# PKU-EPIC/GraspNeRF

Hardware: AMD Instinct MI355X
Metric: scenes/sec TSDF+render fwd, 6-view 40^3 grid (higher is better)
Workload: dtype f32

## Files before the change

graspnerf_amd/_lib.py:

```python
import ctypes as C
import os

_HERE = os.path.dirname(os.path.abspath(__file__))
LIB_PATH = os.path.join(_HERE, 'csrc', os.environ.get('GNR_LIB', 'libgnr.so'))

GNR_OK, GNR_ERR_ARG, GNR_ERR_SHAPE, GNR_ERR_HIP, GNR_ERR_WORKSPACE = 0, -1, -2, -3, -4
ERRORS = {-1: 'GNR_ERR_ARG', -2: 'GNR_ERR_SHAPE', -3: 'GNR_ERR_HIP', -4: 'GNR_ERR_WORKSPACE'}

c_float_p = C.POINTER(C.c_float)


class GnrScene(C.Structure):
    _fields_ = [('B', C.c_int), ('V', C.c_int), ('H', C.c_int), ('W', C.c_int), ('fh', C.c_int), ('fw', C.c_int),
                ('imgs', C.c_void_p), ('img_feats', C.c_void_p), ('ray_feats', C.c_void_p),
                ('poses', C.c_void_p), ('Ks', C.c_void_p), ('depth_range', C.c_void_p), ('use_vis', C.c_int), ('options', C.c_uint)]


OPTIONS = {'fp32_chain': 0x001, 'feature_grad_fixed': 0x002, 'view1_one_wavefront': 0x004, 'view2_one_wavefront': 0x008,
           'ray_order_morton': 0x010, 'poison_partials': 0x020, 'direct_scatter': 0x040, 'geo_dual_fp32': 0x080, 'test_lose_partner': 0x100, 'static_tiles': 0x200, 'split_launch': 0x400}
GNR_STATUS_LOST_PARTNER = 16


class GnrRays(C.Structure):
    _fields_ = [('rn', C.c_int), ('dn', C.c_int), ('fdn', C.c_int),
                ('ray_mask_view_num', C.c_int), ('ray_mask_point_num', C.c_int),
                ('coords', C.c_void_p), ('que_pose', C.c_void_p), ('que_K', C.c_void_p),
                ('que_depth_range', C.c_void_p), ('que_imgs', C.c_void_p), ('fine_u', C.c_void_p),
                ('ray_batch_num', C.c_int), ('fine_depth_use_all', C.c_int)]


RENDER_OUT_FIELDS = ['depth', 'sdf_values', 'alpha_values', 'colors_nr', 'hit_prob_nr', 'pixel_colors_nr',
                     'pixel_colors_gt', 'render_depth', 'ray_mask', 'sdf_gradient_error', 'sdf_gradient', 'view_mask']


# ... 51 lines not shown
    L.gnr_status_words_offset.restype = C.c_size_t
    L.gnr_sample_volume_fwd.argtypes = [C.POINTER(GnrScene), C.c_void_p, C.c_int, C.c_void_p, C.c_void_p,
                                        C.c_void_p, C.c_void_p, C.c_size_t, C.c_void_p]
    L.gnr_sample_volume_fwd.restype = C.c_int
    L.gnr_debug_volume_chain.argtypes = [C.POINTER(GnrScene), C.c_void_p, C.c_int, C.c_void_p, C.c_void_p,
                                         C.c_void_p, C.c_size_t, C.c_void_p]
    L.gnr_debug_volume_chain.restype = C.c_int
    L.gnr_depth_mean_fwd.argtypes = [C.POINTER(GnrScene), C.c_void_p, C.c_int, C.c_void_p, C.c_void_p,
                                     C.c_void_p, C.c_size_t, C.c_void_p]
    L.gnr_depth_mean_fwd.restype = C.c_int
    L.gnr_merge_depths.argtypes = [C.c_void_p, C.c_int, C.c_void_p, C.c_int, C.c_void_p, C.c_int, C.c_void_p]
    L.gnr_merge_depths.restype = C.c_int
    L.gnr_render_by_depth_fwd.argtypes = [C.POINTER(GnrScene), C.POINTER(GnrRays), C.c_void_p, C.c_int, C.c_void_p,
                                          C.POINTER(GnrRenderOut), C.c_void_p, C.c_size_t, C.c_void_p]
    L.gnr_render_by_depth_fwd.restype = C.c_int
    L.gnr_render_rays_fwd.argtypes = [C.POINTER(GnrScene), C.POINTER(GnrRays), C.c_void_p, C.c_void_p,
                                      C.POINTER(GnrRenderOut), C.POINTER(GnrRenderOut), C.c_void_p, C.c_void_p,
                                      C.c_void_p, C.c_size_t, C.c_void_p]
    L.gnr_render_rays_fwd.restype = C.c_int
    L.gnr_head_canonical_floats.restype = C.c_int
    L.gnr_head_packed_floats.restype = C.c_int
    L.gnr_pack_grasp_head.argtypes = [c_float_p, c_float_p]
    L.gnr_pack_grasp_head.restype = C.c_int
    L.gnr_grasp_head_workspace_bytes.argtypes = [C.c_int, C.c_int]
    L.gnr_grasp_head_workspace_bytes.restype = C.c_size_t
    L.gnr_grasp_head_fwd.argtypes = [C.c_int, C.c_int, C.c_void_p, C.c_void_p, C.c_void_p, C.c_void_p, C.c_void_p,
                                     C.c_void_p, C.c_size_t, C.c_void_p]
    L.gnr_grasp_head_fwd.restype = C.c_int
    L.gnr_head_last_error.restype = C.c_char_p
    L.gnr_conv3d_bwd_weight.argtypes = [C.c_void_p] * 3 + [C.c_int] * 7 + [C.c_void_p]
# ... 88 lines not shown
    for fn in (L.gnr_reflect_pad2d, L.gnr_reflect_pad2d_bwd):
        fn.argtypes = [C.c_void_p, C.c_void_p, C.c_longlong, C.c_int, C.c_int, C.c_int, C.c_void_p]
        fn.restype = C.c_int
    L.gnr_upsample2x_bilinear.argtypes = [C.c_void_p, C.c_void_p, C.c_longlong, C.c_int, C.c_int, C.c_void_p]
    L.gnr_upsample2x_bilinear.restype = C.c_int
    L.gnr_last_error.restype = C.c_char_p
    L.gnr_dominant_kernel_name.restype = C.c_char_p
    L.gnr_debug_fill_lds.argtypes = [C.c_uint, C.c_void_p]
    L.gnr_debug_fill_lds.restype = C.c_int
    _lib = L
    return L


EXPORTED = ['gnr_canonical_weights_floats', 'gnr_packed_weights_floats', 'gnr_pack_weights', 'gnr_pack_vis_decoder', 'gnr_pack_vis_decoder_bwd', 'gnr_canonical_vis_floats', 'gnr_pack_weights_device', 'gnr_pack_weights_bwd_device', 'gnr_pack_vis_decoder_device', 'gnr_pack_vis_decoder_bwd_device', 'gnr_layout_offset', 'gnr_workspace_bytes',
            'gnr_prepare', 'gnr_range_status', 'gnr_status_words_offset', 'gnr_sample_volume_fwd', 'gnr_debug_volume_chain', 'gnr_depth_mean_fwd', 'gnr_merge_depths', 'gnr_render_by_depth_fwd', 'gnr_render_rays_fwd',
            'gnr_dominant_kernel_name', 'gnr_last_error', 'gnr_time_chain_kernel', 'gnr_head_canonical_floats',
            'gnr_head_packed_floats', 'gnr_pack_grasp_head', 'gnr_grasp_head_workspace_bytes', 'gnr_grasp_head_fwd',
            'gnr_head_last_error', 'gnr_chain_timing_begin', 'gnr_chain_timing_end', 'gnr_timing_begin', 'gnr_timing_begin_only', 'gnr_timing_end', 'gnr_grasp_select_workspace_bytes',
            'gnr_grasp_select_fwd', 'gnr_post_last_error', 'gnr_packed_bwd_floats', 'gnr_pack_weights_bwd',
            'gnr_depth_mean_bwd_workspace_bytes', 'gnr_depth_mean_bwd', 'gnr_sample_volume_train_workspace_bytes',
            'gnr_train_workspace_layout', 'gnr_sample_volume_fwd_train', 'gnr_sample_volume_bwd',
            'gnr_render_chain_train_workspace_bytes', 'gnr_render_chain_fwd_train', 'gnr_render_chain_bwd', 'gnr_conv3d_bwd_weight', 'gnr_conv3d_same_workspace_bytes', 'gnr_conv3d_same', 'gnr_conv3d_tap_mask_words', 'gnr_conv3d_tap_mask', 'gnr_conv3d_same_masked', 'gnr_conv3d_same_bwd_weight_masked', 'gnr_conv3d_same_bwd_weight', 'gnr_conv3d_same_bwd_weight_workspace_bytes',
            'gnr_render_tail_fwd_train', 'gnr_ray_tail_grad_floats', 'gnr_ray_tail_dual_bwd', 'gnr_ray_tail_dual_bwd_workspace_bytes', 'gnr_composite_bwd', 'gnr_composite_bwd_workspace_bytes', 'gnr_geo_dual_fwd', 'gnr_geo_dual_fwd_workspace_bytes', 'gnr_geo_dual_bwd', 'gnr_geo_dual_bwd_workspace_bytes', 'gnr_host_randperm_prefix',
            'gnr_debug_fill_lds', 'gnr_img_last_error', 'gnr_instnorm_act', 'gnr_instnorm_act_bwd', 'gnr_reflect_pad2d', 'gnr_reflect_pad2d_bwd', 'gnr_upsample2x_bilinear']


def check(rc, what):
    if rc != GNR_OK:
        msg = lib().gnr_last_error().decode(errors='replace')
        raise GnrError(f'{what} failed: {ERRORS.get(rc, rc)} ({msg})')
# ... 17 lines not shown
```

graspnerf_amd/csrc/gnr_capi.inc:

```
#include <stdio.h>
#include <string.h>
#include <atomic>
#include <mutex>

#include "../../include/gnr.h"

namespace gnr {

static thread_local char g_err[512] = "";
static int fail(int code, const char* what, hipError_t e = hipSuccess) {
    snprintf(g_err, sizeof(g_err), "%s%s%s", what, e != hipSuccess ? ": " : "", e != hipSuccess ? hipGetErrorString(e) : "");
    return code;
}
#define GNR_HIP(call)                                                         \
    do {                                                                      \
        hipError_t e_ = (call);                                               \
        if (e_ != hipSuccess) return fail(GNR_ERR_HIP, #call, e_);            \
    } while (0)

static inline size_t al256(size_t x) { return (x + 255) & ~(size_t)255; }

static bool attr_needed(std::atomic<unsigned long long>& done) {
    int dev = 0;
    if (hipGetDevice(&dev) != hipSuccess) return true;
    const unsigned long long bit = 1ull << (dev & 63);
    if (done.load() & bit) return false;
    done.fetch_or(bit);
    return true;
}

struct Workspace {
    float* feat64; float* viewp; unsigned* range_flag;
    float* desc; float* rec; float* depth_c; float* depth_f; float* depth_m; float* gerr_part; unsigned char* vmask_pts;
    int* ray_perm;
    size_t total;
};

static Workspace carve(const GnrScene* s, size_t P, size_t rn, void* base) {
    Workspace w;
    char* p = (char*)base;
    size_t off = 0;
    const size_t BV = (size_t)s->B * s->V;
    auto take = [&](size_t bytes) { char* q = p ? p + off : nullptr; off += al256(bytes); return q; };
    w.feat64 = (float*)take(BV * s->fh * s->fw * 64 * sizeof(float));
    w.viewp = (float*)take(BV * VIEWP_FLOATS * sizeof(float));
    w.range_flag = (unsigned*)take(512);
    w.desc = (float*)take((size_t)s->B * P * DESC_FLOATS * sizeof(float));
    w.rec = (float*)take((size_t)s->B * P * REC_RAY * sizeof(float));
    w.depth_c = (float*)take((size_t)s->B * P * sizeof(float));
    w.depth_f = (float*)take((size_t)s->B * P * sizeof(float));
    w.depth_m = (float*)take((size_t)s->B * P * sizeof(float));
    w.gerr_part = (float*)take((size_t)s->B * (rn > 0 ? rn : 1) * sizeof(float));
    w.vmask_pts = (unsigned char*)take((size_t)s->B * P);
    w.ray_perm = (int*)take((size_t)s->B * (rn > 0 ? rn : 1) * sizeof(int));
    w.total = off;
    return w;
}

enum StatusSlot { RS_SCENE = 0, RS_VOLUME = 1, RS_COARSE = 2, RS_FINE = 3, RS_VOLUME_TRAIN = 4, RS_COARSE_TRAIN = 5, RS_DEPTHS_TRAIN = 6,
                  RS_BACKWARD = 61 , RS_RAY_WATCH = 62 ,
                  RS_FEAT_FX = 63 , RS_WORDS = 64 };
static_assert(RS_DEPTHS_TRAIN < RS_BACKWARD && RS_FEAT_FX < RS_WORDS, "status slots");
static inline bool opt(const GnrScene* s, unsigned bit) { return (s->options & bit) != 0; }

static int check_scene(const GnrScene* s) {
    if (!s || !s->imgs || !s->img_feats || !s->ray_feats || !s->poses || !s->Ks || !s->depth_range)
        return fail(GNR_ERR_ARG, "GnrScene: null pointer");
    if (s->options & ~GNR_OPT_ALL) return fail(GNR_ERR_ARG, "GnrScene.options: unknown bits (GNR_OPT_*)");
    if (s->B < 1 || s->H < 2 || s->W < 2 || s->fh < 1 || s->fw < 1) return fail(GNR_ERR_SHAPE, "GnrScene: bad dims");
// ... 442 lines not shown
    if (!bbox_min || !wc || !dbg || !ws) return fail(GNR_ERR_ARG, "gnr_debug_volume_chain: null pointer");
    return volume_impl(s, bbox_min, R, wc, nullptr, nullptr, ws, ws_bytes, (hipStream_t)stream, true, true, false, dbg);
}

static int order_rays(const GnrScene* s, const GnrRays* q, Workspace& w, hipStream_t st, const int** perm_out) {
    *perm_out = nullptr;
    if (!opt(s, GNR_OPT_RAY_ORDER_MORTON) || q->rn > MAX_SORT_RAYS || q->rn < 2) return GNR_OK;
    int shift = 0;
    while (((s->W > s->H ? s->W : s->H) >> shift) > 1024) ++shift;
    { KScope ks("k_ray_order@render_pass", st); hipLaunchKernelGGL(k_ray_order, dim3(s->B), dim3(256), 0, st, q->coords, w.ray_perm, q->rn, shift); }
    GNR_HIP(hipGetLastError());
    *perm_out = w.ray_perm;
    return GNR_OK;
}

static int render_pass(const GnrScene* s, const GnrRays* q, const float* depth, int dn, const float* wl, GnrRenderOut* out,
                       Workspace& w, hipStream_t st, float* fine_depth, int* fine_inds, int fdn, const float* fine_u = nullptr,
                       const int* perm = nullptr, int range_slot = RS_COARSE, float* gt_also = nullptr, bool skip_gt = false, bool gen_depth = false) {
    if (!out || !out->colors_nr) return fail(GNR_ERR_ARG, "GnrRenderOut.colors_nr is required");
    const int B = s->B, rn = q->rn;
    const int P = rn * dn;
    { KScope ks("k_points_rays@render_pass", st); hipLaunchKernelGGL(k_points_rays, dim3((B * P + 255) / 256), dim3(256), 0, st, q->coords, q->que_pose, q->que_K,
                       q->que_depth_range, depth, w.desc, rn, dn, B, perm, gen_depth ? const_cast<float*>(depth) : nullptr); }
    GNR_HIP(hipGetLastError());
    ChainArgs a{wl, w.feat64, s->imgs, w.viewp, w.desc, w.rec, out->colors_nr, out->view_mask, nullptr,
                B, P, s->H, s->W, s->fh, s->fw, 0};
    a.range_flag = w.range_flag;
    a.range_launch = w.range_flag ? w.range_flag + range_slot : nullptr;
    a.tile_ctr = (w.range_flag && !opt(s, GNR_OPT_STATIC_TILES)) ? w.range_flag + RS_WORDS : nullptr;
    a.ray_perm = perm; a.perm_rn = rn; a.perm_dn = dn;
    if (int rc = launch_chain<true>(s, a, st)) return rc;
    RayArgs r;
    memset(&r, 0, sizeof(r));
    r.wpk = wl; r.rec = w.rec; r.desc = w.desc; r.depth = depth; r.colors = out->colors_nr; r.que_dr = q->que_depth_range;
    r.nrays = B * rn; r.dn = dn; r.rays_per_scene = rn;
    r.sdf = out->sdf_values; r.alpha = out->alpha_values; r.hit = out->hit_prob_nr; r.pix = out->pixel_colors_nr;
    r.rdepth = out->render_depth; r.gerr_part = out->sdf_gradient_error ? w.gerr_part : nullptr; r.grad = out->sdf_gradient;
    r.rmask = out->ray_mask; r.view_num = q->ray_mask_view_num; r.point_num = q->ray_mask_point_num;
    r.fine_depth = fine_depth; r.fine_inds = fine_inds; r.fdn = fdn; r.fine_u = fine_u; r.ray_perm = perm;
    r.range_word = w.range_flag ? w.range_flag + RS_RAY_WATCH : nullptr;
    if (int rc = launch_ray<true>(r, st)) return rc;
    if (out->sdf_gradient_error) {
        const int chunk = q->ray_batch_num > 0 ? q->ray_batch_num : rn;
        { KScope ks("k_gerr_reduce@render_pass", st); hipLaunchKernelGGL(k_gerr_reduce, dim3(B, (rn + chunk - 1) / chunk), dim3(256), 0, st, w.gerr_part,
                           out->sdf_gradient_error, rn, dn, chunk); }
// ... 18 lines not shown
    return GNR_OK;
}

extern "C" int gnr_render_by_depth_fwd(const GnrScene* s, const GnrRays* q, const float* depth, int dn, const float* wl,
                                       GnrRenderOut* out, void* ws, size_t ws_bytes, void* stream) {
    if (int rc = check_scene(s)) return rc;
    if (int rc = check_rays(q, true)) return rc;
    if (!depth || !wl || !ws) return fail(GNR_ERR_ARG, "gnr_render_by_depth_fwd: null pointer");
    if (dn < 3 || dn > MAX_DN_FWD) return fail(GNR_ERR_SHAPE, "dn must be in 3..128");
    if (int rc = check_points(s, (size_t)q->rn * dn)) return rc;
    Workspace w = carve(s, (size_t)q->rn * dn, q->rn, ws);
    if (ws_bytes < w.total) return fail(GNR_ERR_WORKSPACE, "workspace too small");
    const int* perm = nullptr;
    if (int rc = order_rays(s, q, w, (hipStream_t)stream, &perm)) return rc;
    return render_pass(s, q, depth, dn, wl, out, w, (hipStream_t)stream, nullptr, nullptr, 0, nullptr, perm);
}

extern "C" int gnr_render_rays_fwd(const GnrScene* s, const GnrRays* q, const float* wc, const float* wf, GnrRenderOut* coarse,
                                   GnrRenderOut* fine, const float* fine_depth_in, int* fine_inds_out, void* ws, size_t ws_bytes,
                                   void* stream) {
    if (int rc = check_scene(s)) return rc;
    if (int rc = check_rays(q)) return rc;
    if (!wc || !coarse || !ws || (fine && !wf)) return fail(GNR_ERR_ARG, "gnr_render_rays_fwd: null pointer");
    if (!fine && (fine_depth_in || fine_inds_out)) return fail(GNR_ERR_ARG, "gnr_render_rays_fwd: fine depths / indices without a fine pass");
    hipStream_t st = (hipStream_t)stream;
    const int fine_dn = !fine ? 0 : (q->fine_depth_use_all ? q->dn + q->fdn : q->fdn);
    const int dmax = q->dn > fine_dn ? q->dn : fine_dn;
    if (int rc = check_points(s, (size_t)q->rn * dmax)) return rc;
    Workspace w = carve(s, (size_t)q->rn * dmax, q->rn, ws);
    if (ws_bytes < w.total) return fail(GNR_ERR_WORKSPACE, "workspace too small");
// ... 767 lines not shown
```

graspnerf_amd/csrc/gnr_kernels.hip:

```cpp
#include <hip/hip_runtime.h>
#include <stdint.h>
#include <type_traits>

#include "gnr_layout.h"

#ifndef GNR_ABLATE
#define GNR_ABLATE 0
#endif

namespace gnr {

typedef float f4 __attribute__((ext_vector_type(4)));
typedef float f2 __attribute__((ext_vector_type(2)));

#define DEV __device__ __forceinline__

DEV f4 mfma16(float a, float b, f4 c) { return __builtin_amdgcn_mfma_f32_16x16x4f32(a, b, c, 0, 0, 0); }
DEV float elu1(float x) { return fmaxf(x, __builtin_amdgcn_fmed3f(__expf(x), 0.f, 1.f) - 1.f); }
constexpr float kLog2e = 1.4426950408889634f, kLn2 = 0.6931471805599453f;
#if GNR_ABLATE & 8
DEV float elu_s(float xs) { return xs; }
#else
DEV float elu_s(float xs) { return fmaxf(xs, fmaf(__builtin_amdgcn_fmed3f(__builtin_amdgcn_exp2f(xs), 0.f, 1.f), kLog2e, -kLog2e)); }
#endif
// ... 377 lines not shown
    for (int k2 = 2; k2 <= M; k2 <<= 1)
        for (int j = k2 >> 1; j > 0; j >>= 1) {
            for (int i = threadIdx.x; i < M; i += 256) {
                const int l = i ^ j;
                if (l > i) {
                    const unsigned a = key[i], c = key[l];
                    const bool up = (i & k2) == 0;
                    if ((a > c) == up) { key[i] = c; key[l] = a; }
                }
            }
            __syncthreads();
        }
    for (int i = threadIdx.x; i < rn; i += 256) perm[(size_t)b * rn + i] = (int)(key[i] & 0xFFFu);
}

__global__ void k_points_rays(const float* __restrict__ coords, const float* __restrict__ que_pose,
                              const float* __restrict__ que_K, const float* __restrict__ que_dr,
                              const float* __restrict__ depth, float* __restrict__ desc, int rn, int dn, int B,
                              const int* __restrict__ perm = nullptr, float* __restrict__ depth_gen = nullptr) {
    const int i = blockIdx.x * blockDim.x + threadIdx.x;
    if (i >= B * rn * dn) return;
    const int b = i / (rn * dn), slot = (i / dn) % rn, k = i % dn;
    const int ray = perm ? perm[(size_t)b * rn + slot] : slot;
    const float* P = que_pose + b * 12;
    float Ki[9];
    inv3x3(que_K + b * 9, Ki);
    const float u = coords[((size_t)b * rn + ray) * 2], v = coords[((size_t)b * rn + ray) * 2 + 1];
    float cam[3], tr[3], dir[3];
    for (int r = 0; r < 3; ++r) cam[r] = Ki[r * 3] * u + Ki[r * 3 + 1] * v + Ki[r * 3 + 2];
    for (int c = 0; c < 3; ++c) tr[c] = -(P[c] * P[3] + P[4 + c] * P[7] + P[8 + c] * P[11]);
    for (int c = 0; c < 3; ++c) {
        const float rc = P[c] * cam[0] + P[4 + c] * cam[1] + P[8 + c] * cam[2];
        dir[c] = __fsub_rn(__fadd_rn(rc, tr[c]), tr[c]);
    }
// ... 2 lines not shown
    auto z = [&](int j) -> float {
        if (!depth_gen) return zp[j];
        const float diff = __fsub_rn(__fdiv_rn(1.f, dfar), __fdiv_rn(1.f, dnear));
        float tick = __fmul_rn(__fdiv_rn(diff, (float)(dn - 1)), (float)j);
        if (j == 0) tick = 0.f;
        if (j == dn - 1) tick = diff;
        return __fdiv_rn(1.f, __fadd_rn(__fdiv_rn(1.f, dnear), tick));
    };
    const float zk = z(k);
    if (depth_gen) depth_gen[((size_t)b * rn + ray) * dn + k] = zk;
    const float nrm = sqrtf(dir[0] * dir[0] + dir[1] * dir[1] + dir[2] * dir[2]);
    const float near = -1.f / dnear, far = -1.f / dfar;
    auto inv = [&](int j) { return __fdiv_rn(__fsub_rn(__fdiv_rn(-1.f, z(j)), near), __fsub_rn(far, near)); };
    auto half = [&](int j) { return (j == dn - 1) ? 0.5e6f : __fmul_rn(__fsub_rn(inv(j + 1), inv(j)), 0.5f); };
    float* d = desc + (size_t)i * DESC_FLOATS;
    for (int c = 0; c < 3; ++c) {
        d[c] = tr[c] + dir[c] * zk;
        d[3 + c] = -dir[c] / nrm;
    }
    d[6] = half(k == 0 ? 0 : k - 1);
    d[7] = half(k);
}

__global__ void k_desc_unpack(const float* __restrict__ desc, float* __restrict__ pts, float* __restrict__ qdir, int dn, int n) {
    const int i = blockIdx.x * blockDim.x + threadIdx.x;
    if (i >= n) return;
    const float* d = desc + (size_t)i * DESC_FLOATS;
    if (pts) { pts[(size_t)i * 3] = d[0]; pts[(size_t)i * 3 + 1] = d[1]; pts[(size_t)i * 3 + 2] = d[2]; }
    if (qdir && i % dn == 0) { float* q = qdir + (size_t)(i / dn) * 3; q[0] = d[3]; q[1] = d[4]; q[2] = d[5]; }
}

struct ChainArgs {
    const float* wpk;
    const float* feat64;
    const float* imgs;
    const float* viewp;
    const float* desc;
    float* rec;
    float* colors;
    unsigned char* vmask;
    float* dbg;
    int B, P, H, W, fh, fw;
    int vol_res;
    float* save1;
    float* save2;
    float* saveG;
    float* saveZ;
    unsigned* range_flag;
    int only_if_flagged;
    unsigned* range_launch;
    const int* ray_perm; int perm_rn, perm_dn;
    unsigned* tile_ctr;
    const float* bbox_min;
    int pts_R;
    int b0;
};

struct ViewGeom {
    float u, v, z, m;
    float dd[4];
};

template <bool FULL>
DEV void project_view(const float* __restrict__ vp, const float (&p)[3], const float (&qd)[3], int H, int W, ViewGeom& o) {
    const float pcx = __fmaf_rn(vp[2], p[2], __fmaf_rn(vp[1], p[1], __fmul_rn(vp[0], p[0]))) + vp[3];
    const float pcy = __fmaf_rn(vp[6], p[2], __fmaf_rn(vp[5], p[1], __fmul_rn(vp[4], p[0]))) + vp[7];
// ... 75 lines not shown
    d[0] *= inr; d[1] *= inr; d[2] *= inr;
    dd[0] = d[0] - qd[0]; dd[1] = d[1] - qd[1]; dd[2] = d[2] - qd[2];
    dd[3] = d[0] * qd[0] + d[1] * qd[1] + d[2] * qd[2];
}

constexpr int SW = 20;
#ifndef GNR_TWO_QUEUES
#define GNR_TWO_QUEUES 0
#endif
#ifndef GNR_RDF2_PAIRS
#define GNR_RDF2_PAIRS 0
#endif
constexpr int rows_a(int V) { return GNR_TWO_QUEUES ? (V + 1) / 2 : V; }
constexpr int rows_b(int V) { return GNR_TWO_QUEUES ? V / 2 : 0; }

#ifndef GNR_DYN_TILES
#define GNR_DYN_TILES 1
#endif
#ifndef GNR_VOLUME_POINTS_INLINE
#define GNR_VOLUME_POINTS_INLINE 1
#endif
#ifndef GNR_TAIL_OLD_ONLY
#define GNR_TAIL_OLD_ONLY 0
#endif
#ifndef GNR_DESC_PREFETCH
#define GNR_DESC_PREFETCH 0
#endif
#ifndef GNR_DYN_CTR_INC
#define GNR_DYN_CTR_INC 0
#endif
// ... 106 lines not shown
#endif
    };
    auto locate = [&](int tile_, int& b_, int& ts_) {
        b_ = tile_ / tps;
        ts_ = tile_ - b_ * tps;
        b_ += a.b0;
        if (a.vol_res > 0) {
            const int R = a.vol_res, tpg = R >> 3, gpr = R >> 1;
            const int BX = R >> 2, GY = R >> 3, GB = BX * GY;
            const int sidx = ts_ / tpg, tin = ts_ - sidx * tpg;
            const int brick = sidx / GB, wi = sidx - brick * GB;
            const int bx = brick >> 2, by = brick & 3;
            ts_ = ((BX * bx + wi / GY) * gpr + GY * by + wi % GY) * tpg + tin;
        }
    };
    auto point_of = [&](int b_, int ts_) -> size_t { const int nr = ts_ * 16 + r; return (size_t)b_ * a.P + (nr < a.P ? nr : a.P - 1); };
    int tile = dyn ? resolve(grab()) : xcd * chunk + lblk * waves_per_block + wave;
    constexpr bool DPF = GNR_DESC_PREFETCH != 0 && !SAVE;
    f4 d0n = {0.f, 0.f, 0.f, 0.f}, d1n = d0n;
    bool have_nxt = false;
    for (; dyn ? tile >= 0 : tile < t_end;) {
        GNR_ITER_FENCE();
        unsigned tile_nxt = 0u;
        int tile_after = -1;
#if GNR_WAVE_CLOCK
        const unsigned long long wc_tt = wall_clock64();
#endif
        int b, ts;
        locate(tile, b, ts);
        const int n_raw = ts * 16 + r;
        const bool row_ok = n_raw < a.P;
        const int n = row_ok ? n_raw : a.P - 1;
        const size_t pt = (size_t)b * a.P + n;
        size_t opt = pt;
        if (RENDER && !SAVE && a.ray_perm) {
            const int s_ = n / a.perm_dn;
            opt = (size_t)b * a.P + (size_t)a.ray_perm[(size_t)b * a.perm_rn + s_] * a.perm_dn + (n - s_ * a.perm_dn);
        }
        float p[3], qd[3], lo, hi;
        {
            f4 d0, d1;
            if (DPF && have_nxt) { d0 = d0n; d1 = d1n; }
            else if (!RENDER && !SAVE && GNR_VOLUME_POINTS_INLINE != 0 && a.pts_R > 0) {
                const int R = a.pts_R;
                const float invR = 1.f / (float)R;
                const int col = (int)(((float)n + 0.5f) * invR), sz = n - col * R;
                const int ix = (int)(((float)col + 0.5f) * invR), iy = col - ix * R, iz = R - 1 - sz;
// ... 1244 lines not shown
```

graspnerf_amd/hotpath.py:

```python
import ctypes as C

import numpy as np
import torch

from . import _lib
from ._lib import GnrScene, GnrRays, GnrRenderOut

RENDER_KEYS = ['sdf_values', 'alpha_values', 'colors_nr', 'hit_prob_nr', 'pixel_colors_nr', 'pixel_colors_gt',
               'render_depth', 'ray_mask', 'sdf_gradient_error']


def _f32(t, device):
    if not torch.is_tensor(t):
        t = torch.as_tensor(np.asarray(t))
    return t.to(device=device, dtype=torch.float32).contiguous()


class HotPath:
    default_options = 0

    def __init__(self, packed_coarse, packed_fine=None, device='cuda:0'):
        self.L = _lib.lib()
        if not torch.cuda.is_available():
            raise _lib.GnrError('graspnerf_amd hot path needs a ROCm GPU (torch.cuda.is_available() is False); '
# ... 159 lines not shown
        scene, keep, ws = prepared or self.prepare(ref, 1, rn, max(dn, fine_dn))
        rays, rkeep = self._rays(que, dn, fdn, cfg, scene.H, scene.W)
        co_s, co = self._alloc_out(B, rn, dn, 'imgs' in que, debug, rays.ray_batch_num)
        fi_s, fi = self._alloc_out(B, rn, fine_dn, 'imgs' in que, debug, rays.ray_batch_num)
        fd_in = _f32(fine_depth_in, self.device) if fine_depth_in is not None else None
        inds = torch.empty(B, rn, fdn, dtype=torch.int32, device=self.device) if debug else None
        _lib.check(self.L.gnr_render_rays_fwd(self._sc(scene), C.byref(rays), self.wc.data_ptr(), self.wf.data_ptr(),
                                              C.byref(co_s), C.byref(fi_s),
                                              fd_in.data_ptr() if fd_in is not None else None,
                                              inds.data_ptr() if debug else None,
                                              ws.data_ptr(), ws.numel(), self._stream()), 'gnr_render_rays_fwd')
        for o in (co, fi):
            o['ray_mask'] = o['ray_mask'].view(torch.bool)
        return (co, fi, inds) if debug else (co, fi)

    def render_by_depth(self, ref, que, depth, level='coarse', cfg=None, debug=False, prepared=None):
        cfg = cfg or {}
        depth = _f32(depth, self.device)
        B, rn, dn = depth.shape
        scene, keep, ws = prepared or self.prepare(ref, 1, rn, dn)
        rays, rkeep = self._rays(que, dn, dn, cfg, scene.H, scene.W)
        o_s, o = self._alloc_out(B, rn, dn, 'imgs' in que, debug, rays.ray_batch_num)
        w = self.wc if level == 'coarse' else self.wf
        _lib.check(self.L.gnr_render_by_depth_fwd(self._sc(scene), C.byref(rays), depth.data_ptr(), dn, w.data_ptr(),
                                                  C.byref(o_s), ws.data_ptr(), ws.numel(), self._stream()),
                   'gnr_render_by_depth_fwd')
        o['ray_mask'] = o['ray_mask'].view(torch.bool)
        return o

    def merge_depths(self, a, b):
        a, b = _f32(a, self.device), _f32(b, self.device)
        assert a.shape[:-1] == b.shape[:-1]
        out = torch.empty(*a.shape[:-1], a.shape[-1] + b.shape[-1], dtype=torch.float32, device=self.device)
        _lib.check(self.L.gnr_merge_depths(a.data_ptr(), a.shape[-1], b.data_ptr(), b.shape[-1], out.data_ptr(), a.numel() // a.shape[-1],
                                           self._stream()), 'gnr_merge_depths')
        return out

    def depth_mean(self, ref, coords, level='coarse', prepared=None):
        scene, keep, ws = prepared or self.prepare(ref, 1)
        coords = _f32(coords, self.device)
        B, pn, _ = coords.shape
        out = torch.empty(B, scene.V, pn, 2, dtype=torch.float32, device=self.device)
        w = self.wc if level == 'coarse' else self.wf
# ... 207 lines not shown
```

include/gnr.h:

```cpp
#ifndef GNR_H
#define GNR_H
#include <stddef.h>

#ifdef __cplusplus
extern "C" {
#endif

#define GNR_OK 0
#define GNR_ERR_ARG (-1)
#define GNR_ERR_SHAPE (-2)
#define GNR_ERR_HIP (-3)
#define GNR_ERR_WORKSPACE (-4)

typedef struct GnrScene {
    int B, V;
    int H, W;
    int fh, fw;
    const float* imgs;
    const float* img_feats;
    const float* ray_feats;
    const float* poses;
    const float* Ks;
    const float* depth_range;
    int use_vis;
    unsigned options;
} GnrScene;

#define GNR_OPT_FP32_CHAIN 0x001u
#define GNR_OPT_FEATURE_GRAD_FIXED 0x002u
#define GNR_OPT_VIEW1_ONE_WAVEFRONT 0x004u
#define GNR_OPT_VIEW2_ONE_WAVEFRONT 0x008u
#define GNR_OPT_RAY_ORDER_MORTON 0x010u
#define GNR_OPT_POISON_PARTIALS 0x020u
#define GNR_OPT_DIRECT_SCATTER 0x040u
#define GNR_OPT_GEO_DUAL_FP32 0x080u
#define GNR_OPT_TEST_LOSE_PARTNER 0x100u
#define GNR_OPT_STATIC_TILES 0x200u
#define GNR_OPT_SPLIT_LAUNCH 0x400u
#define GNR_OPT_ALL 0x7ffu

typedef struct GnrRays {
    int rn;
    int dn;
    int fdn;
    int ray_mask_view_num;
    int ray_mask_point_num;
    const float* coords;
    const float* que_pose;
    const float* que_K;
    const float* que_depth_range;
    const float* que_imgs;
    const float* fine_u;
    int ray_batch_num;
    int fine_depth_use_all;
// ... 35 lines not shown
size_t gnr_status_words_offset(const GnrScene* scene);

int gnr_sample_volume_fwd(const GnrScene* scene, const float* bbox_min , int volume_res,
                          const float* packed_coarse , float* sdf_out ,
                          unsigned char* view_mask_out, void* workspace, size_t workspace_bytes,
                          void* stream);

int gnr_render_by_depth_fwd(const GnrScene* scene, const GnrRays* rays, const float* depth, int dn,
                            const float* level_weights, GnrRenderOut* out, void* workspace,
                            size_t workspace_bytes, void* stream);

int gnr_render_rays_fwd(const GnrScene* scene, const GnrRays* rays, const float* packed_coarse,
                        const float* packed_fine, GnrRenderOut* coarse, GnrRenderOut* fine,
                        const float* fine_depth_in, int* fine_inds_out, void* workspace,
                        size_t workspace_bytes, void* stream);

int gnr_merge_depths(const float* depth_a, int na, const float* depth_b, int nb, float* out, int nrays, void* stream);

int gnr_depth_mean_fwd(const GnrScene* scene, const float* coords, int pn, const float* level_weights,
                       float* mean_out, void* workspace, size_t workspace_bytes, void* stream);

int gnr_debug_volume_chain(const GnrScene* scene, const float* bbox_min, int volume_res,
                           const float* packed_coarse, float* dbg, void* workspace,
                           size_t workspace_bytes, void* stream);

int gnr_head_canonical_floats(void);
int gnr_head_packed_floats(void);
int gnr_pack_grasp_head(const float* canonical_host, float* packed_host);
size_t gnr_grasp_head_workspace_bytes(int B, int volume_res);
int gnr_grasp_head_fwd(int B, int volume_res, const float* volume, const float* packed_head, float* qual, float* rot,
// ... 115 lines not shown
```

Measured before the change: 5078.

## Reorder render samples by view-visibility mask to cut wavefront divergence

New measurement: 5157, median of 6. 1.02x the previous value.

```diff
diff --git a/graspnerf_amd/_lib.py b/graspnerf_amd/_lib.py
--- a/graspnerf_amd/_lib.py
+++ b/graspnerf_amd/_lib.py
@@ -17,7 +17,8 @@
 
 
 OPTIONS = {'fp32_chain': 0x001, 'feature_grad_fixed': 0x002, 'view1_one_wavefront': 0x004, 'view2_one_wavefront': 0x008,
-           'ray_order_morton': 0x010, 'poison_partials': 0x020, 'direct_scatter': 0x040, 'geo_dual_fp32': 0x080, 'test_lose_partner': 0x100, 'static_tiles': 0x200, 'split_launch': 0x400}
+           'ray_order_morton': 0x010, 'poison_partials': 0x020, 'direct_scatter': 0x040, 'geo_dual_fp32': 0x080, 'test_lose_partner': 0x100, 'static_tiles': 0x200, 'split_launch': 0x400,
+           'sample_order_natural': 0x800}
 GNR_STATUS_LOST_PARTNER = 16
 
 
@@ -99,6 +100,15 @@
     L.gnr_render_by_depth_fwd.argtypes = [C.POINTER(GnrScene), C.POINTER(GnrRays), C.c_void_p, C.c_int, C.c_void_p,
                                           C.POINTER(GnrRenderOut), C.c_void_p, C.c_size_t, C.c_void_p]
     L.gnr_render_by_depth_fwd.restype = C.c_int
+    L.gnr_debug_render_by_depth_perm.argtypes = [C.POINTER(GnrScene), C.POINTER(GnrRays), C.c_void_p, C.c_int, C.c_void_p,
+                                                 C.POINTER(GnrRenderOut), C.c_void_p, C.c_void_p, C.c_size_t, C.c_void_p]
+    L.gnr_debug_render_by_depth_perm.restype = C.c_int
+    L.gnr_debug_sample_order.argtypes = [C.c_void_p, C.c_int, C.c_int, C.c_void_p, C.c_void_p]
+    L.gnr_debug_sample_order.restype = C.c_int
+    L.gnr_sample_order_host.argtypes = [C.c_void_p, C.c_int, C.c_void_p]
+    L.gnr_sample_order_host.restype = C.c_int
+    L.gnr_sample_order_offsets.argtypes = [C.POINTER(GnrScene), C.c_int, C.c_int, C.POINTER(C.c_size_t), C.POINTER(C.c_size_t)]
+    L.gnr_sample_order_offsets.restype = C.c_int
     L.gnr_render_rays_fwd.argtypes = [C.POINTER(GnrScene), C.POINTER(GnrRays), C.c_void_p, C.c_void_p,
                                       C.POINTER(GnrRenderOut), C.POINTER(GnrRenderOut), C.c_void_p, C.c_void_p,
                                       C.c_void_p, C.c_size_t, C.c_void_p]
@@ -217,6 +227,7 @@
 
 EXPORTED = ['gnr_canonical_weights_floats', 'gnr_packed_weights_floats', 'gnr_pack_weights', 'gnr_pack_vis_decoder', 'gnr_pack_vis_decoder_bwd', 'gnr_canonical_vis_floats', 'gnr_pack_weights_device', 'gnr_pack_weights_bwd_device', 'gnr_pack_vis_decoder_device', 'gnr_pack_vis_decoder_bwd_device', 'gnr_layout_offset', 'gnr_workspace_bytes',
             'gnr_prepare', 'gnr_range_status', 'gnr_status_words_offset', 'gnr_sample_volume_fwd', 'gnr_debug_volume_chain', 'gnr_depth_mean_fwd', 'gnr_merge_depths', 'gnr_render_by_depth_fwd', 'gnr_render_rays_fwd',
+            'gnr_debug_render_by_depth_perm', 'gnr_debug_sample_order', 'gnr_sample_order_host', 'gnr_sample_order_offsets',
             'gnr_dominant_kernel_name', 'gnr_last_error', 'gnr_time_chain_kernel', 'gnr_head_canonical_floats',
             'gnr_head_packed_floats', 'gnr_pack_grasp_head', 'gnr_grasp_head_workspace_bytes', 'gnr_grasp_head_fwd',
             'gnr_head_last_error', 'gnr_chain_timing_begin', 'gnr_chain_timing_end', 'gnr_timing_begin', 'gnr_timing_begin_only', 'gnr_timing_end', 'gnr_grasp_select_workspace_bytes',
diff --git a/graspnerf_amd/csrc/gnr_capi.inc b/graspnerf_amd/csrc/gnr_capi.inc
--- a/graspnerf_amd/csrc/gnr_capi.inc
+++ b/graspnerf_amd/csrc/gnr_capi.inc
@@ -33,6 +33,7 @@
     float* feat64; float* viewp; unsigned* range_flag;
     float* desc; float* rec; float* depth_c; float* depth_f; float* depth_m; float* gerr_part; unsigned char* vmask_pts;
     int* ray_perm;
+    int* sample_perm; unsigned char* sample_keys;
     size_t total;
 };
 
@@ -53,6 +54,8 @@
     w.gerr_part = (float*)take((size_t)s->B * (rn > 0 ? rn : 1) * sizeof(float));
     w.vmask_pts = (unsigned char*)take((size_t)s->B * P);
     w.ray_perm = (int*)take((size_t)s->B * (rn > 0 ? rn : 1) * sizeof(int));
+    w.sample_perm = rn > 0 ? (int*)take((size_t)s->B * P * sizeof(int)) : nullptr;
+    w.sample_keys = rn > 0 ? (unsigned char*)take((size_t)s->B * P) : nullptr;
     w.total = off;
     return w;
 }
@@ -525,21 +528,38 @@
     return GNR_OK;
 }
 
+constexpr int SAMPLE_ORDER_MIN_TILES_PER_SLOT = 8;
+static bool sample_order_wanted(const GnrScene* s, const Workspace& w, int P) {
+    if (opt(s, GNR_OPT_SAMPLE_ORDER_NATURAL) || !w.sample_perm || !w.sample_keys || P > MAX_SORT_SAMPLES) return false;
+    const long ntiles = (long)s->B * ((P + 15) / 16), slots = (long)num_cus() * (GNR_CHAIN_THREADS / 64);
+    return ntiles >= SAMPLE_ORDER_MIN_TILES_PER_SLOT * slots;
+}
+static int launch_sample_order(const unsigned char* keys, int* perm, int B, int P, int nkeys, hipStream_t st) {
+    { KScope ks("k_sample_order@render_pass", st); hipLaunchKernelGGL(k_sample_order, dim3(B), dim3(1024), 0, st, keys, perm, P, nkeys); }
+    GNR_HIP(hipGetLastError());
+    return GNR_OK;
+}
 static int render_pass(const GnrScene* s, const GnrRays* q, const float* depth, int dn, const float* wl, GnrRenderOut* out,
                        Workspace& w, hipStream_t st, float* fine_depth, int* fine_inds, int fdn, const float* fine_u = nullptr,
-                       const int* perm = nullptr, int range_slot = RS_COARSE, float* gt_also = nullptr, bool skip_gt = false, bool gen_depth = false) {
+                       const int* perm = nullptr, int range_slot = RS_COARSE, float* gt_also = nullptr, bool skip_gt = false, bool gen_depth = false,
+                       const int* sample_perm_in = nullptr) {
     if (!out || !out->colors_nr) return fail(GNR_ERR_ARG, "GnrRenderOut.colors_nr is required");
     const int B = s->B, rn = q->rn;
     const int P = rn * dn;
+    const bool ordered = !sample_perm_in && sample_order_wanted(s, w, P);
     { KScope ks("k_points_rays@render_pass", st); hipLaunchKernelGGL(k_points_rays, dim3((B * P + 255) / 256), dim3(256), 0, st, q->coords, q->que_pose, q->que_K,
-                       q->que_depth_range, depth, w.desc, rn, dn, B, perm, gen_depth ? const_cast<float*>(depth) : nullptr); }
-    GNR_HIP(hipGetLastError());
+                       q->que_depth_range, depth, w.desc, rn, dn, B, perm, gen_depth ? const_cast<float*>(depth) : nullptr,
+                       ordered ? w.sample_keys : nullptr, w.viewp, s->V, s->H, s->W); }
+    GNR_HIP(hipGetLastError());
+    if (ordered)
+        if (int rc = launch_sample_order(w.sample_keys, w.sample_perm, B, P, 1 << s->V, st)) return rc;
     ChainArgs a{wl, w.feat64, s->imgs, w.viewp, w.desc, w.rec, out->colors_nr, out->view_mask, nullptr,
                 B, P, s->H, s->W, s->fh, s->fw, 0};
     a.range_flag = w.range_flag;
     a.range_launch = w.range_flag ? w.range_flag + range_slot : nullptr;
     a.tile_ctr = (w.range_flag && !opt(s, GNR_OPT_STATIC_TILES)) ? w.range_flag + RS_WORDS : nullptr;
     a.ray_perm = perm; a.perm_rn = rn; a.perm_dn = dn;
+    a.sample_perm = ordered ? w.sample_perm : sample_perm_in;
     if (int rc = launch_chain<true>(s, a, st)) return rc;
     RayArgs r;
     memset(&r, 0, sizeof(r));
@@ -588,6 +608,47 @@
     const int* perm = nullptr;
     if (int rc = order_rays(s, q, w, (hipStream_t)stream, &perm)) return rc;
     return render_pass(s, q, depth, dn, wl, out, w, (hipStream_t)stream, nullptr, nullptr, 0, nullptr, perm);
+}
+
+extern "C" int gnr_debug_render_by_depth_perm(const GnrScene* s, const GnrRays* q, const float* depth, int dn, const float* wl,
+                                              GnrRenderOut* out, const int* sample_perm, void* ws, size_t ws_bytes, void* stream) {
+    if (int rc = check_scene(s)) return rc;
+    if (int rc = check_rays(q, true)) return rc;
+    if (!depth || !wl || !ws || !sample_perm) return fail(GNR_ERR_ARG, "gnr_debug_render_by_depth_perm: null pointer");
+    if (dn < 3 || dn > MAX_DN_FWD) return fail(GNR_ERR_SHAPE, "dn must be in 3..128");
+    if (int rc = check_points(s, (size_t)q->rn * dn)) return rc;
+    Workspace w = carve(s, (size_t)q->rn * dn, q->rn, ws);
+    if (ws_bytes < w.total) return fail(GNR_ERR_WORKSPACE, "workspace too small");
+    const int* perm = nullptr;
+    if (int rc = order_rays(s, q, w, (hipStream_t)stream, &perm)) return rc;
+    return render_pass(s, q, depth, dn, wl, out, w, (hipStream_t)stream, nullptr, nullptr, 0, nullptr, perm, RS_COARSE, nullptr, false, false, sample_perm);
+}
+
+extern "C" int gnr_debug_sample_order(const unsigned char* keys, int B, int P, int* perm, void* stream) {
+    if (!keys || !perm) return fail(GNR_ERR_ARG, "gnr_debug_sample_order: null pointer");
+    if (B < 1 || P < 1 || P > MAX_SORT_SAMPLES) return fail(GNR_ERR_SHAPE, "gnr_debug_sample_order: 1 <= P <= 2^18 samples per scene");
+    return launch_sample_order(keys, perm, B, P, 256, (hipStream_t)stream);
+}
+extern "C" int gnr_sample_order_host(const unsigned char* keys, int P, int* perm_out) {
+    if (!keys || !perm_out) return fail(GNR_ERR_ARG, "gnr_sample_order_host: null pointer");
+    if (P < 1) return fail(GNR_ERR_SHAPE, "gnr_sample_order_host: P must be positive");
+    int start[256], hist[256] = {0};
+    for (int i = 0; i < P; ++i) ++hist[keys[i]];
+    for (int k = 0; k < 256; ++k) {
+        start[k] = 0;
+        for (int k2 = 0; k2 < 256; ++k2) if (sorder::key_before(k2, k)) start[k] += hist[k2];
+    }
+    for (int i = 0; i < P; ++i) perm_out[sorder::slot_of(start[keys[i]]++, P)] = i;
+    return GNR_OK;
+}
+extern "C" int gnr_sample_order_offsets(const GnrScene* s, int rn, int dn_max, size_t* keys_off, size_t* perm_off) {
+    if (!s || !keys_off || !perm_off) return fail(GNR_ERR_ARG, "gnr_sample_order_offsets: null pointer");
+    if (rn < 1 || dn_max < 1) return fail(GNR_ERR_SHAPE, "gnr_sample_order_offsets: rn, dn_max must be positive");
+    char* const base = (char*)4096;
+    Workspace w = carve(s, (size_t)rn * dn_max, rn, base);
+    if ((size_t)rn * dn_max > (size_t)MAX_SORT_SAMPLES) return fail(GNR_ERR_SHAPE, "gnr_sample_order_offsets: more samples per scene than the sort handles");
+    *keys_off = (size_t)((char*)w.sample_keys - base); *perm_off = (size_t)((char*)w.sample_perm - base);
+    return GNR_OK;
 }
 
 extern "C" int gnr_render_rays_fwd(const GnrScene* s, const GnrRays* q, const float* wc, const float* wf, GnrRenderOut* coarse,
diff --git a/graspnerf_amd/csrc/gnr_kernels.hip b/graspnerf_amd/csrc/gnr_kernels.hip
--- a/graspnerf_amd/csrc/gnr_kernels.hip
+++ b/graspnerf_amd/csrc/gnr_kernels.hip
@@ -3,6 +3,7 @@
 #include <type_traits>
 
 #include "gnr_layout.h"
+#include "gnr_sample_order.h"
 
 #ifndef GNR_ABLATE
 #define GNR_ABLATE 0
@@ -415,10 +416,13 @@
     for (int i = threadIdx.x; i < rn; i += 256) perm[(size_t)b * rn + i] = (int)(key[i] & 0xFFFu);
 }
 
+DEV unsigned view_mask_key(const float* __restrict__ viewp_b, const float (&p)[3], int V, int H, int W);
+
 __global__ void k_points_rays(const float* __restrict__ coords, const float* __restrict__ que_pose,
                               const float* __restrict__ que_K, const float* __restrict__ que_dr,
                               const float* __restrict__ depth, float* __restrict__ desc, int rn, int dn, int B,
-                              const int* __restrict__ perm = nullptr, float* __restrict__ depth_gen = nullptr) {
+                              const int* __restrict__ perm = nullptr, float* __restrict__ depth_gen = nullptr,
+                              unsigned char* __restrict__ keys = nullptr, const float* __restrict__ viewp = nullptr, int V = 0, int H = 0, int W = 0) {
     const int i = blockIdx.x * blockDim.x + threadIdx.x;
     if (i >= B * rn * dn) return;
     const int b = i / (rn * dn), slot = (i / dn) % rn, k = i % dn;
@@ -451,12 +455,15 @@
     auto inv = [&](int j) { return __fdiv_rn(__fsub_rn(__fdiv_rn(-1.f, z(j)), near), __fsub_rn(far, near)); };
     auto half = [&](int j) { return (j == dn - 1) ? 0.5e6f : __fmul_rn(__fsub_rn(inv(j + 1), inv(j)), 0.5f); };
     float* d = desc + (size_t)i * DESC_FLOATS;
+    float pw[3];
     for (int c = 0; c < 3; ++c) {
-        d[c] = tr[c] + dir[c] * zk;
+        pw[c] = tr[c] + dir[c] * zk;
+        d[c] = pw[c];
         d[3 + c] = -dir[c] / nrm;
     }
     d[6] = half(k == 0 ? 0 : k - 1);
     d[7] = half(k);
+    if (keys) keys[i] = (unsigned char)view_mask_key(viewp + (size_t)b * V * VIEWP_FLOATS, pw, V, H, W);
 }
 
 __global__ void k_desc_unpack(const float* __restrict__ desc, float* __restrict__ pts, float* __restrict__ qdir, int dn, int n) {
@@ -487,6 +494,7 @@
     int only_if_flagged;
     unsigned* range_launch;
     const int* ray_perm; int perm_rn, perm_dn;
+    const int* sample_perm;
     unsigned* tile_ctr;
     const float* bbox_min;
     int pts_R;
@@ -592,6 +600,75 @@
 constexpr int rows_a(int V) { return GNR_TWO_QUEUES ? (V + 1) / 2 : V; }
 constexpr int rows_b(int V) { return GNR_TWO_QUEUES ? V / 2 : 0; }
 
+DEV unsigned view_mask_key(const float* __restrict__ viewp_b, const float (&p)[3], int V, int H, int W) {
+    const float qd[3] = {0.f, 0.f, 0.f};
+    unsigned k = 0;
+    for (int v = 0; v < V; ++v) {
+        ViewGeom vg;
+        project_view<false>(viewp_b + v * VIEWP_FLOATS, p, qd, H, W, vg);
+        k |= (vg.m != 0.f ? 1u : 0u) << v;
+    }
+    return k;
+}
+constexpr int MAX_SORT_SAMPLES = 1 << 18;
+constexpr int SO_DEPTH = 16;
+__global__ __launch_bounds__(1024) void k_sample_order(const unsigned char* __restrict__ keys, int* __restrict__ perm, int P, int nkeys) {
+    __shared__ int hist[256];
+    __shared__ int wbase[16][256];
+    const int tid = threadIdx.x, lane = tid & 63, wave = tid >> 6;
+    const unsigned char* kb = keys + (size_t)blockIdx.x * P;
+    int* pb = perm + (size_t)blockIdx.x * P;
+    for (int i = tid; i < 16 * 256; i += 1024) (&wbase[0][0])[i] = 0;
+    __syncthreads();
+    const int seg = ((P + 16 * 64 - 1) / (16 * 64)) * 64;
+    const int s0 = min(P, wave * seg), s1 = min(P, s0 + seg);
+    for (int i0 = s0; i0 < s1; i0 += 64 * SO_DEPTH) {
+        int kk[SO_DEPTH];
+#pragma unroll
+        for (int u = 0; u < SO_DEPTH; ++u) { const int i = i0 + u * 64 + lane; kk[u] = i < s1 ? (int)kb[i] : -1; }
+#pragma unroll
+        for (int u = 0; u < SO_DEPTH; ++u) if (kk[u] >= 0) atomicAdd(&wbase[wave][kk[u]], 1);
+    }
+    __syncthreads();
+    if (tid < nkeys) {
+        int t = 0;
+        for (int w = 0; w < 16; ++w) t += wbase[w][tid];
+        hist[tid] = t;
+    }
+    __syncthreads();
+    if (tid < nkeys) {
+        int run = 0;
+        for (int k2 = 0; k2 < nkeys; ++k2) if (sorder::key_before(k2, tid)) run += hist[k2];
+        for (int w = 0; w < 16; ++w) { const int c = wbase[w][tid]; wbase[w][tid] = run; run += c; }
+    }
+    __syncthreads();
+    volatile int* base = wbase[wave];
+    for (int i0 = s0; i0 < s1; i0 += 64 * SO_DEPTH) {
+        int kk[SO_DEPTH];
+#pragma unroll
+        for (int u = 0; u < SO_DEPTH; ++u) { const int i = i0 + u * 64 + lane; kk[u] = i < s1 ? (int)kb[i] : -1; }
+#pragma unroll
+        for (int u = 0; u < SO_DEPTH; ++u) {
+            if (i0 + u * 64 >= s1) break;
+            const int k = kk[u];
+            const bool ok = k >= 0;
+            unsigned long long same = __ballot(ok);
+#pragma unroll
+            for (int bit = 0; bit < 8; ++bit) {
+                const bool on = (k >> bit) & 1;
+                const unsigned long long bb = __ballot(on);
+                same &= on ? bb : ~bb;
+            }
+            const int rank = __popcll(same & ((1ull << lane) - 1ull));
+            const int pos = ok ? base[k] + rank : 0;
+            __builtin_amdgcn_wave_barrier();
+            if (ok && rank == 0) base[k] = pos + __popcll(same);
+            __builtin_amdgcn_wave_barrier();
+            if (ok) pb[sorder::slot_of(pos, P)] = i0 + u * 64 + lane;
+        }
+    }
+}
+
 #ifndef GNR_DYN_TILES
 #define GNR_DYN_TILES 1
 #endif
@@ -728,7 +805,11 @@
             ts_ = ((BX * bx + wi / GY) * gpr + GY * by + wi % GY) * tpg + tin;
         }
     };
-    auto point_of = [&](int b_, int ts_) -> size_t { const int nr = ts_ * 16 + r; return (size_t)b_ * a.P + (nr < a.P ? nr : a.P - 1); };
+    auto point_of = [&](int b_, int ts_) -> size_t {
+        int nr = min(ts_ * 16 + r, a.P - 1);
+        if (RENDER && !SAVE && a.sample_perm) nr = min(max(a.sample_perm[(size_t)b_ * a.P + nr], 0), a.P - 1);
+        return (size_t)b_ * a.P + nr;
+    };
     int tile = dyn ? resolve(grab()) : xcd * chunk + lblk * waves_per_block + wave;
     constexpr bool DPF = GNR_DESC_PREFETCH != 0 && !SAVE;
     f4 d0n = {0.f, 0.f, 0.f, 0.f}, d1n = d0n;
@@ -744,7 +825,10 @@
         locate(tile, b, ts);
         const int n_raw = ts * 16 + r;
         const bool row_ok = n_raw < a.P;
-        const int n = row_ok ? n_raw : a.P - 1;
+        int n = row_ok ? n_raw : a.P - 1;
+        if constexpr (RENDER && !SAVE) {
+            if (a.sample_perm) n = min(max(a.sample_perm[(size_t)b * a.P + n], 0), a.P - 1);
+        }
         const size_t pt = (size_t)b * a.P + n;
         size_t opt = pt;
         if (RENDER && !SAVE && a.ray_perm) {
diff --git a/graspnerf_amd/csrc/gnr_sample_order.h b/graspnerf_amd/csrc/gnr_sample_order.h
--- /dev/null
+++ b/graspnerf_amd/csrc/gnr_sample_order.h
@@ -0,0 +1,39 @@
+#pragma once
+
+#if defined(__HIPCC__)
+#define GNR_SO_HD __host__ __device__
+#else
+#define GNR_SO_HD
+#endif
+
+namespace gnr {
+namespace sorder {
+
+constexpr int STRIPES = 8;
+constexpr int TILE = 16;
+
+GNR_SO_HD inline int popcount8(int k) { k = (k & 0x55) + ((k >> 1) & 0x55); k = (k & 0x33) + ((k >> 2) & 0x33); return (k & 0x0f) + (k >> 4); }
+
+GNR_SO_HD inline bool key_before(int a, int b) {
+    const int pa = popcount8(a), pb = popcount8(b);
+    return pa != pb ? pa > pb : a > b;
+}
+
+GNR_SO_HD inline int stripe_tiles(int tps, int s) { return (tps - s + STRIPES - 1) / STRIPES; }
+
+GNR_SO_HD inline int slot_of(int pos, int P) {
+    const int tps = (P + TILE - 1) / TILE;
+    const int rem = P - (tps - 1) * TILE;
+    const int gshort = tps <= STRIPES ? tps - 1 : STRIPES * (tps / STRIPES) - 1;
+    int gi, wi;
+    if (pos < TILE * gshort) { gi = pos / TILE; wi = pos % TILE; }
+    else if (pos < TILE * gshort + rem) { gi = gshort; wi = pos - TILE * gshort; }
+    else { const int q = pos + TILE - rem; gi = q / TILE; wi = q % TILE; }
+    const int s = gi % STRIPES;
+    int tile = gi / STRIPES;
+    for (int k = 0; k < s; ++k) tile += stripe_tiles(tps, k);
+    return tile * TILE + wi;
+}
+
+}
+}
diff --git a/graspnerf_amd/hotpath.py b/graspnerf_amd/hotpath.py
--- a/graspnerf_amd/hotpath.py
+++ b/graspnerf_amd/hotpath.py
@@ -197,7 +197,7 @@
             o['ray_mask'] = o['ray_mask'].view(torch.bool)
         return (co, fi, inds) if debug else (co, fi)
 
-    def render_by_depth(self, ref, que, depth, level='coarse', cfg=None, debug=False, prepared=None):
+    def render_by_depth(self, ref, que, depth, level='coarse', cfg=None, debug=False, prepared=None, _sample_perm=None):
         cfg = cfg or {}
         depth = _f32(depth, self.device)
         B, rn, dn = depth.shape
@@ -205,11 +205,35 @@
         rays, rkeep = self._rays(que, dn, dn, cfg, scene.H, scene.W)
         o_s, o = self._alloc_out(B, rn, dn, 'imgs' in que, debug, rays.ray_batch_num)
         w = self.wc if level == 'coarse' else self.wf
-        _lib.check(self.L.gnr_render_by_depth_fwd(self._sc(scene), C.byref(rays), depth.data_ptr(), dn, w.data_ptr(),
-                                                  C.byref(o_s), ws.data_ptr(), ws.numel(), self._stream()),
-                   'gnr_render_by_depth_fwd')
+        if _sample_perm is not None:
+            sp = _sample_perm.to(device=self.device, dtype=torch.int32).contiguous()
+            assert sp.shape == (B, rn * dn)
+            _lib.check(self.L.gnr_debug_render_by_depth_perm(self._sc(scene), C.byref(rays), depth.data_ptr(), dn, w.data_ptr(), C.byref(o_s),
+                                                             sp.data_ptr(), ws.data_ptr(), ws.numel(), self._stream()),
+                       'gnr_debug_render_by_depth_perm')
+        else:
+            _lib.check(self.L.gnr_render_by_depth_fwd(self._sc(scene), C.byref(rays), depth.data_ptr(), dn, w.data_ptr(),
+                                                      C.byref(o_s), ws.data_ptr(), ws.numel(), self._stream()),
+                       'gnr_render_by_depth_fwd')
         o['ray_mask'] = o['ray_mask'].view(torch.bool)
         return o
+
+    def debug_render_by_depth_perm(self, ref, que, depth, sample_perm, level='coarse', cfg=None, debug=False, prepared=None):
+        return self.render_by_depth(ref, que, depth, level, cfg, debug, prepared, _sample_perm=sample_perm)
+
+    def sample_order_state(self, rn, dn_max, P, prepared=None):
+        scene, keep, ws = prepared or self._prepared
+        ko, po = C.c_size_t(0), C.c_size_t(0)
+        _lib.check(self.L.gnr_sample_order_offsets(self._sc(scene), rn, dn_max, C.byref(ko), C.byref(po)), 'gnr_sample_order_offsets')
+        B = scene.B
+        return ws[ko.value:ko.value + B * P].view(B, P), ws[po.value:po.value + 4 * B * P].view(torch.int32).view(B, P)
+
+    def debug_sample_order(self, keys):
+        keys = keys.to(device=self.device, dtype=torch.uint8).contiguous()
+        B, P = keys.shape
+        perm = torch.empty(B, P, dtype=torch.int32, device=self.device)
+        _lib.check(self.L.gnr_debug_sample_order(keys.data_ptr(), B, P, perm.data_ptr(), self._stream()), 'gnr_debug_sample_order')
+        return perm
 
     def merge_depths(self, a, b):
         a, b = _f32(a, self.device), _f32(b, self.device)
diff --git a/include/gnr.h b/include/gnr.h
--- a/include/gnr.h
+++ b/include/gnr.h
@@ -37,7 +37,8 @@
 #define GNR_OPT_TEST_LOSE_PARTNER 0x100u
 #define GNR_OPT_STATIC_TILES 0x200u
 #define GNR_OPT_SPLIT_LAUNCH 0x400u
-#define GNR_OPT_ALL 0x7ffu
+#define GNR_OPT_SAMPLE_ORDER_NATURAL 0x800u
+#define GNR_OPT_ALL 0xfffu
 
 typedef struct GnrRays {
     int rn;
@@ -103,6 +104,12 @@
                         const float* packed_fine, GnrRenderOut* coarse, GnrRenderOut* fine,
                         const float* fine_depth_in, int* fine_inds_out, void* workspace,
                         size_t workspace_bytes, void* stream);
+
+int gnr_debug_render_by_depth_perm(const GnrScene* scene, const GnrRays* rays, const float* depth, int dn, const float* level_weights,
+                                   GnrRenderOut* out, const int* sample_perm, void* workspace, size_t workspace_bytes, void* stream);
+int gnr_debug_sample_order(const unsigned char* keys, int B, int P, int* perm, void* stream);
+int gnr_sample_order_host(const unsigned char* keys_host, int P, int* perm_out_host);
+int gnr_sample_order_offsets(const GnrScene* scene, int rn, int dn_max, size_t* keys_offset, size_t* perm_offset);
 
 int gnr_merge_depths(const float* depth_a, int na, const float* depth_b, int nb, float* out, int nrays, void* stream);
 
```
